# christophersanborn/Radiative3D

Hardware: AMD Instinct MI355X
Metric: phonon-histories/sec (higher is better)
Workload: dtype f64

## Files before the change

### radiative3d_amd/csrc/r3d_tables_build.h

```cpp
#ifndef R3D_TABLES_BUILD_H_
#define R3D_TABLES_BUILD_H_

#include <hip/hip_runtime.h>

#include <cstdint>

#include "r3d_tables.h"

namespace r3d {

hipError_t build_scatterer_tables(const double het[6], double psdf_numer, const double* d_toa, uint64_t n,
                                  double* d_cdf[4], double* d_spol, double totals[4], double cos_sums[4],
                                  hipStream_t stream);

hipError_t build_toa_on_device(int degree, uint64_t n, double* d_toa, hipStream_t stream);
hipError_t build_toa_xyz_on_device(const double* d_toa, uint64_t n, double min_theta, double max_theta,
                                   double* d_xyz, hipStream_t stream);
hipError_t build_source_tables(const double moment[6], const double* d_toa, uint64_t n, double* d_cdf[3],
                               double totals[3], hipStream_t stream);

hipError_t build_spol_cs_on_device(const double* d_spol, uint64_t n, double* d_cs, hipStream_t stream);

hipError_t build_guide_on_device(const double* d_cdf, uint64_t n, uint32_t bits, GuideCell* d_guide,
                                 hipStream_t stream);

}
#endif
```

### radiative3d_amd/csrc/r3d_tables_build.hip

```cpp
#include <hip/hip_runtime.h>

#include <cmath>
#include <cstdint>
#include <vector>

#include "r3d_tables_build.h"

namespace r3d {

namespace {

constexpr int kThreads = 256;
constexpr int kItems = 16;
constexpr int kScanBlock = kThreads * kItems;

struct Het {
  double nu, eps, a, kappa, el, gam0, psdf_numer;
};

__device__ __forceinline__ double psato(const Het& h, double m) {
  return h.psdf_numer / pow(1. + h.a * h.a * m * m, h.kappa + 1.5);
}

__global__ __launch_bounds__(kThreads) void gsato_kernel(Het h, const double* __restrict__ toa, uint64_t n,
                                                         double* __restrict__ w0, double* __restrict__ w1,
                                                         double* __restrict__ w2, double* __restrict__ w3,
                                                         double* __restrict__ spol,
                                                         double* __restrict__ block_cos ) {
  const uint64_t k = (uint64_t)blockIdx.x * kThreads + threadIdx.x;
  double g[4] = {0, 0, 0, 0}, cz = 0;
  if (k < n) {
    const double psi = toa[2 * k], zeta = toa[2 * k + 1];
    const double g2 = h.gam0 * h.gam0;
    const double cpsi = cos(psi), c2psi = cos(2. * psi), spsi = sin(psi);
    const double czeta = cos(zeta), szeta = sin(zeta);
    const double spsi2 = spsi * spsi;
    const double xpp = (1. / g2) * (h.nu * (-1. + cpsi + (2. / g2) * spsi2) - 2. + (4. / g2) * spsi2);
    const double xps = -spsi * (h.nu * (1. - (2. / h.gam0) * cpsi) - (4. / h.gam0) * cpsi);
    const double xsp = (1. / g2) * spsi * czeta * (h.nu * (1. - (2. / h.gam0) * cpsi) - (4. / h.gam0) * cpsi);
    const double xss_psi = czeta * (h.nu * (cpsi - c2psi) - 2. * c2psi);
    const double xss_zeta = szeta * (h.nu * (cpsi - 1.) + 2. * cpsi);
    const double pi4 = 4. * 3.14159265358979323846;
    const double el4 = (h.el * h.el) * (h.el * h.el);
    double m = (2. * h.el / h.gam0) * sin(psi / 2.);
    g[0] = (el4 / pi4) * (xpp * xpp) * psato(h, m);
    m = (h.el / h.gam0) * sqrt(1. + g2 - 2. * h.gam0 * cpsi);
    const double pm = psato(h, m);
    g[1] = (1. / h.gam0) * (el4 / pi4) * (xps * xps) * pm;
    g[2] = h.gam0 * (el4 / pi4) * (xsp * xsp) * pm;
    m = 2. * h.el * sin(psi / 2.);
    g[3] = (el4 / pi4) * (xss_psi * xss_psi + xss_zeta * xss_zeta) * psato(h, m);
#pragma unroll
    for (int c = 0; c < 4; c++)
      if (g[c] < 1.e-30) g[c] = 0.;
    w0[k] = g[0], w1[k] = g[1], w2[k] = g[2], w3[k] = g[3];
    spol[k] = atan2(xss_zeta, xss_psi);
    cz = cpsi;
  }
  __shared__ double s_part[kThreads / 64][4];
#pragma unroll
  for (int c = 0; c < 4; c++) {
    double v = cz * g[c];
#pragma unroll
    for (int off = 32; off > 0; off >>= 1) v += __shfl_xor(v, off);
    if ((threadIdx.x & 63) == 0) s_part[threadIdx.x >> 6][c] = v;
  }
  __syncthreads();
  if (threadIdx.x < 4) {
    double v = 0;
    for (int wv = 0; wv < kThreads / 64; wv++) v += s_part[wv][threadIdx.x];
    block_cos[(size_t)blockIdx.x * 4 + threadIdx.x] = v;
  }
}

__global__ __launch_bounds__(kThreads) void scan_blocks(double* const* __restrict__ arrays, uint64_t n,
                                                        double* __restrict__ block_sums, uint32_t n_blocks) {
  double* v = arrays[blockIdx.y];
  const uint64_t base = (uint64_t)blockIdx.x * kScanBlock + (uint64_t)threadIdx.x * kItems;
  double x[kItems];
  double run = 0;
#pragma unroll
  for (int i = 0; i < kItems; i++) {
    const uint64_t k = base + i;
    run += (k < n) ? v[k] : 0.0;
    x[i] = run;
  }
  __shared__ double s_run[kThreads];
  s_run[threadIdx.x] = run;
  __syncthreads();
  if (threadIdx.x == 0) {
    double acc = 0;
    for (int t = 0; t < kThreads; t++) {
      const double r = s_run[t];
      s_run[t] = acc;
      acc += r;
    }
  }
  __syncthreads();
  const double before = s_run[threadIdx.x];
#pragma unroll
  for (int i = 0; i < kItems; i++) {
    const uint64_t k = base + i;
    if (k < n) v[k] = before + x[i];
  }
  if (threadIdx.x == kThreads - 1) block_sums[(size_t)blockIdx.y * n_blocks + blockIdx.x] = before + run;
}

__global__ void scan_block_sums(double* __restrict__ block_sums, uint32_t n_blocks) {
  double* s = block_sums + (size_t)blockIdx.x * n_blocks;
  if (threadIdx.x == 0) {
    double run = 0;
    for (uint32_t b = 0; b < n_blocks; b++) {
      const double t = s[b];
      s[b] = run;
      run += t;
    }
  }
}

__global__ __launch_bounds__(kThreads) void add_offsets(double* const* __restrict__ arrays, uint64_t n,
                                                        const double* __restrict__ block_sums, uint32_t n_blocks) {
  double* v = arrays[blockIdx.y];
  const double off = block_sums[(size_t)blockIdx.y * n_blocks + blockIdx.x];
  if (blockIdx.x == 0) return;
  const uint64_t base = (uint64_t)blockIdx.x * kScanBlock;
  for (int i = threadIdx.x; i < kScanBlock; i += kThreads) {
    const uint64_t k = base + i;
    if (k < n) v[k] += off;
  }
}

__device__ uint64_t guide_bound(const double* __restrict__ cdf, uint64_t n, uint64_t j, uint64_t G) {
  const double r = cdf[n - 1] * ((double)j / (double)G);
  uint64_t lo = 0, hi = n - 1;
  while (lo < hi) {
    const uint64_t mid = (lo + hi) >> 1;
    if (r <= cdf[mid]) hi = mid;
    else lo = mid + 1;
  }
  return lo;
}
__global__ __launch_bounds__(kThreads) void guide_kernel(const double* __restrict__ cdf, uint64_t n, uint32_t bits,
                                                         GuideCell* __restrict__ guide) {
  const uint64_t G = 1ull << bits;
  const uint64_t j = (uint64_t)blockIdx.x * kThreads + threadIdx.x;
  if (j >= G) return;
  GuideCell c;
  const uint64_t k1 = guide_bound(cdf, n, j, G), k2 = guide_bound(cdf, n, j + 1, G);
  c.k1 = (uint32_t)k1, c.k2 = (uint32_t)k2;
#pragma unroll
  for (int i = 0; i < kGuideVals; i++)
    c.c[i] = (k2 - k1 <= (uint64_t)kGuideVals) ? cdf[k1 + i < k2 ? k1 + i : k2] : cdf[guide_pivot(k1, k2, i)];
  guide[j] = c;
}

struct P3 {
  double x, y, z;
};
__device__ __forceinline__ P3 unit_sum2(P3 a, P3 b) {
#pragma clang fp contract(off)
  const double sx = a.x + b.x, sy = a.y + b.y, sz = a.z + b.z;
  const double m = sqrt(sx * sx + sy * sy + sz * sz);
  return P3{sx / m, sy / m, sz / m};
}
__global__ __launch_bounds__(kThreads) void toa_kernel(int degree, uint64_t n, double* __restrict__ toa) {
#pragma clang fp contract(off)
  const uint64_t k = (uint64_t)blockIdx.x * kThreads + threadIdx.x;
  if (k >= n) return;
  const double g = (1. + sqrt(5.0)) / 2.0;
  const double m1 = sqrt(1.0 + g * g);
  const double u = 1.0 / m1, w = g / m1;
  const P3 v[12] = {{u, 0, w},  {-u, 0, w}, {u, 0, -w}, {-u, 0, -w}, {w, -u, 0}, {w, u, 0},
                    {-w, -u, 0}, {-w, u, 0}, {0, w, u},  {0, w, -u},  {0, -w, u}, {0, -w, -u}};
  const int face[20][3] = {{0, 1, 10}, {0, 1, 8},  {2, 3, 11}, {2, 3, 9},  {4, 5, 0},  {4, 5, 2},  {7, 6, 1},
                           {7, 6, 3},  {10, 11, 4}, {10, 11, 6}, {8, 9, 5},  {8, 9, 7},  {0, 10, 4}, {0, 8, 5},
                           {1, 10, 6}, {1, 8, 7},  {2, 11, 4}, {2, 9, 5},  {3, 11, 6}, {3, 9, 7}};
  const uint32_t f = (uint32_t)(k >> (2 * degree));
  P3 a = v[face[f][0]], b = v[face[f][1]], c = v[face[f][2]];
  for (int level = degree - 1; level >= 0; level--) {
    const uint32_t d = (uint32_t)(k >> (2 * level)) & 3u;
    const P3 ab = unit_sum2(a, b), bc = unit_sum2(b, c), ca = unit_sum2(c, a);
    if (d == 0) b = ab, c = ca;
    else if (d == 1) a = ab, c = bc;
    else if (d == 2) a = ca, b = bc;
    else a = bc, b = ca, c = ab;
  }
  const double sx = a.x + b.x + c.x, sy = a.y + b.y + c.y, sz = a.z + b.z + c.z;
  const double m = sqrt(sx * sx + sy * sy + sz * sz);
  toa[2 * k] = acos(sz / m);
  toa[2 * k + 1] = atan2(sy / m, sx / m);
}
__global__ __launch_bounds__(kThreads) void toa_xyz_kernel(const double* __restrict__ toa, uint64_t n, double min_theta,
                                                           double max_theta, double* __restrict__ xyz) {
#pragma clang fp contract(off)
  const uint64_t k = (uint64_t)blockIdx.x * kThreads + threadIdx.x;
  if (k >= n) return;
  double th = toa[2 * k];
  const double ph = toa[2 * k + 1];
  if (th < min_theta) th = min_theta;
  if (th > max_theta) th = max_theta;
  xyz[4 * k] = cos(th), xyz[4 * k + 1] = cos(ph), xyz[4 * k + 2] = sin(ph), xyz[4 * k + 3] = sin(th);
}
struct Moment {
  double xx, yy, zz, xy, xz, yz;
};
__global__ __launch_bounds__(kThreads) void source_kernel(Moment mt, const double* __restrict__ toa, uint64_t n,
                                                          double* __restrict__ w0, double* __restrict__ w1,
                                                          double* __restrict__ w2) {
  const uint64_t k = (uint64_t)blockIdx.x * kThreads + threadIdx.x;
  if (k >= n) return;
  const double th = toa[2 * k], az = toa[2 * k + 1];
  const double st = sin(th), ct = cos(th), sa = sin(az), ca = cos(az);
  const double horiz = mt.xx * ca * ca + mt.xy * sin(2 * az) + mt.yy * sa * sa - mt.zz;
  const double vert = mt.xz * ca + mt.yz * sa;
  const double p = st * st * horiz + 2 * st * ct * vert + mt.zz;
  const double sh = st * (0.5 * sin(2 * az) * (mt.yy - mt.xx) + cos(2 * az) * mt.xy) + ct * (ca * mt.yz - sa * mt.xz);
  const double sv = st * ct * horiz + (1.0 - 2 * st * st) * vert;
  w0[k] = p * p, w1[k] = sh * sh, w2[k] = sv * sv;
}

hipError_t scan_arrays(double* const* d_arr, int count, uint64_t n, hipStream_t stream) {
  const uint32_t s_blocks = (uint32_t)((n + kScanBlock - 1) / kScanBlock);
  double* d_sums = nullptr;
  double** d_arrays = nullptr;
  hipError_t err = hipMalloc(&d_sums, (size_t)s_blocks * count * sizeof(double));
  if (err == hipSuccess) err = hipMalloc(&d_arrays, count * sizeof(double*));
  if (err == hipSuccess) err = hipMemcpyAsync(d_arrays, d_arr, count * sizeof(double*), hipMemcpyHostToDevice, stream);
  if (err == hipSuccess) {
    scan_blocks<<<dim3(s_blocks, count), kThreads, 0, stream>>>(d_arrays, n, d_sums, s_blocks);
    scan_block_sums<<<count, 64, 0, stream>>>(d_sums, s_blocks);
    add_offsets<<<dim3(s_blocks, count), kThreads, 0, stream>>>(d_arrays, n, d_sums, s_blocks);
    err = hipGetLastError();
  }
  if (err == hipSuccess) err = hipStreamSynchronize(stream);
  (void)hipFree(d_sums), (void)hipFree(d_arrays);
  return err;
}

}

hipError_t build_toa_on_device(int degree, uint64_t n, double* d_toa, hipStream_t stream) {
  if (degree < 0 || degree > 12 || n != ((uint64_t)20 << (2 * degree))) return hipErrorInvalidValue;
  toa_kernel<<<(uint32_t)((n + kThreads - 1) / kThreads), kThreads, 0, stream>>>(degree, n, d_toa);
  return hipGetLastError();
}

hipError_t build_toa_xyz_on_device(const double* d_toa, uint64_t n, double min_theta, double max_theta,
                                   double* d_xyz, hipStream_t stream) {
  toa_xyz_kernel<<<(uint32_t)((n + kThreads - 1) / kThreads), kThreads, 0, stream>>>(d_toa, n, min_theta, max_theta, d_xyz);
  return hipGetLastError();
}

hipError_t build_source_tables(const double moment[6], const double* d_toa, uint64_t n, double* d_cdf[3],
                               double totals[3], hipStream_t stream) {
  if (n == 0) return hipErrorInvalidValue;
  const Moment mt{moment[0], moment[1], moment[2], moment[3], moment[4], moment[5]};
  source_kernel<<<(uint32_t)((n + kThreads - 1) / kThreads), kThreads, 0, stream>>>(mt, d_toa, n, d_cdf[0], d_cdf[1], d_cdf[2]);
  hipError_t err = hipGetLastError();
  if (err == hipSuccess) err = scan_arrays(d_cdf, 3, n, stream);
  for (int c = 0; c < 3 && err == hipSuccess; c++)
    err = hipMemcpy(&totals[c], d_cdf[c] + (n - 1), sizeof(double), hipMemcpyDeviceToHost);
  return err;
}

hipError_t build_scatterer_tables(const double het[6], double psdf_numer, const double* d_toa, uint64_t n,
                                  double* d_cdf[4], double* d_spol, double totals[4], double cos_sums[4],
                                  hipStream_t stream) {
  if (n == 0) return hipErrorInvalidValue;
  Het h{het[0], het[1], het[2], het[3], het[4], het[5], psdf_numer};
  const uint32_t g_blocks = (uint32_t)((n + kThreads - 1) / kThreads);
  const uint32_t s_blocks = (uint32_t)((n + kScanBlock - 1) / kScanBlock);
  double *d_cos = nullptr, *d_sums = nullptr;
  double** d_arrays = nullptr;
  hipError_t err = hipMalloc(&d_cos, (size_t)g_blocks * 4 * sizeof(double));
  if (err == hipSuccess) err = hipMalloc(&d_sums, (size_t)s_blocks * 4 * sizeof(double));
  if (err == hipSuccess) err = hipMalloc(&d_arrays, 4 * sizeof(double*));
  if (err == hipSuccess) err = hipMemcpyAsync(d_arrays, d_cdf, 4 * sizeof(double*), hipMemcpyHostToDevice, stream);
  if (err == hipSuccess) {
    gsato_kernel<<<g_blocks, kThreads, 0, stream>>>(h, d_toa, n, d_cdf[0], d_cdf[1], d_cdf[2], d_cdf[3], d_spol, d_cos);
    scan_blocks<<<dim3(s_blocks, 4), kThreads, 0, stream>>>(d_arrays, n, d_sums, s_blocks);
    scan_block_sums<<<4, 64, 0, stream>>>(d_sums, s_blocks);
    add_offsets<<<dim3(s_blocks, 4), kThreads, 0, stream>>>(d_arrays, n, d_sums, s_blocks);
    err = hipGetLastError();
  }
  std::vector<double> h_cos((size_t)g_blocks * 4);
  if (err == hipSuccess)
    err = hipMemcpyAsync(h_cos.data(), d_cos, h_cos.size() * sizeof(double), hipMemcpyDeviceToHost, stream);
  for (int c = 0; c < 4 && err == hipSuccess; c++)
    err = hipMemcpyAsync(&totals[c], d_cdf[c] + (n - 1), sizeof(double), hipMemcpyDeviceToHost, stream);
  if (err == hipSuccess) err = hipStreamSynchronize(stream);
  if (err == hipSuccess) {
    for (int c = 0; c < 4; c++) cos_sums[c] = 0;
    for (uint32_t b = 0; b < g_blocks; b++)
      for (int c = 0; c < 4; c++) cos_sums[c] += h_cos[(size_t)b * 4 + c];
  }
  (void)hipFree(d_cos), (void)hipFree(d_sums), (void)hipFree(d_arrays);
  return err;
}

__global__ __launch_bounds__(kThreads) void spol_cs_kernel(const double* __restrict__ spol, uint64_t n,
                                                           double* __restrict__ cs) {
  const uint64_t k = (uint64_t)blockIdx.x * kThreads + threadIdx.x;
  if (k >= n) return;
  double s, c;
  sincos(spol[k], &s, &c);
  cs[2 * k] = c, cs[2 * k + 1] = s;
}
hipError_t build_spol_cs_on_device(const double* d_spol, uint64_t n, double* d_cs, hipStream_t stream) {
  spol_cs_kernel<<<(uint32_t)((n + kThreads - 1) / kThreads), kThreads, 0, stream>>>(d_spol, n, d_cs);
  return hipGetLastError();
}

hipError_t build_guide_on_device(const double* d_cdf, uint64_t n, uint32_t bits, GuideCell* d_guide,
                                 hipStream_t stream) {
  const uint64_t G = 1ull << bits;
  guide_kernel<<<(uint32_t)((G + kThreads - 1) / kThreads), kThreads, 0, stream>>>(d_cdf, n, bits, d_guide);
  return hipGetLastError();
}

}
```

Measured before the change: 1.388 billion.

## Restructure table-build scan and guide construction with LDS staging and wave-parallel search

Replaces the three-kernel scan (local scan, serial block-sum scan, add offsets) with a reduce-then-scan scheme. Loads are coalesced and staged through padded LDS, block offsets come from an LDS-chunked serial chain, and array pointers travel by value instead of through a device copy. The guide builder now locates segment bounds with a 64-lane ballot search, samples the CDF segment into LDS, and writes cells with coalesced 16-byte stores. Host-side syncs and per-total memcpys are merged into one readback. This only touches table setup, so its effect on a histories/sec throughput metric depends on whether setup time is inside the timed region.

```diff
diff --git a/radiative3d_amd/csrc/r3d_tables_build.h b/radiative3d_amd/csrc/r3d_tables_build.h
--- a/radiative3d_amd/csrc/r3d_tables_build.h
+++ b/radiative3d_amd/csrc/r3d_tables_build.h
@@ -19,6 +19,8 @@
 hipError_t build_source_tables(const double moment[6], const double* d_toa, uint64_t n, double* d_cdf[3],
                                double totals[3], hipStream_t stream);
 
+hipError_t scan_arrays(double* const* d_arr, int count, uint64_t n, hipStream_t stream);
+
 hipError_t build_spol_cs_on_device(const double* d_spol, uint64_t n, double* d_cs, hipStream_t stream);
 
 hipError_t build_guide_on_device(const double* d_cdf, uint64_t n, uint32_t bits, GuideCell* d_guide,
diff --git a/radiative3d_amd/csrc/r3d_tables_build.hip b/radiative3d_amd/csrc/r3d_tables_build.hip
--- a/radiative3d_amd/csrc/r3d_tables_build.hip
+++ b/radiative3d_amd/csrc/r3d_tables_build.hip
@@ -73,85 +73,181 @@
   }
 }
 
-__global__ __launch_bounds__(kThreads) void scan_blocks(double* const* __restrict__ arrays, uint64_t n,
-                                                        double* __restrict__ block_sums, uint32_t n_blocks) {
-  double* v = arrays[blockIdx.y];
-  const uint64_t base = (uint64_t)blockIdx.x * kScanBlock + (uint64_t)threadIdx.x * kItems;
-  double x[kItems];
+struct ScanArrays {
+  double* v[4];
+};
+constexpr int kScanPad = kScanBlock + kScanBlock / kItems;
+__device__ __forceinline__ int scan_slot(int e) { return e + (e >> 4); }
+
+__device__ __forceinline__ double chain_in_lds(double* s, uint32_t m, double run) {
+  double cur[8], nxt[8];
+#pragma unroll
+  for (int i = 0; i < 8; i++) cur[i] = s[i];
+  for (uint32_t b = 0; b < m; b += 8) {
+#pragma unroll
+    for (int i = 0; i < 8; i++) nxt[i] = s[b + 8 + i];
+#pragma unroll
+    for (int i = 0; i < 8; i++) {
+      s[b + i] = run;
+      run += cur[i];
+      cur[i] = nxt[i];
+    }
+  }
+  return run;
+}
+
+__device__ __forceinline__ double scan_block_runs(const double* __restrict__ v, uint64_t n, double* s_x, double* s_run,
+                                                  double* total) {
+  const uint64_t base = (uint64_t)blockIdx.x * kScanBlock;
+#pragma unroll
+  for (int i = 0; i < kItems; i++) {
+    const int e = i * kThreads + (int)threadIdx.x;
+    const uint64_t k = base + e;
+    s_x[scan_slot(e)] = (k < n) ? v[k] : 0.0;
+  }
+  __syncthreads();
   double run = 0;
 #pragma unroll
+  for (int i = 0; i < kItems; i++) run += s_x[scan_slot((int)threadIdx.x * kItems + i)];
+  s_run[threadIdx.x] = run;
+  if (threadIdx.x < 8) s_run[kThreads + threadIdx.x] = 0;
+  __syncthreads();
+  if (threadIdx.x == 0) s_run[kThreads + 8] = chain_in_lds(s_run, kThreads, 0.0);
+  __syncthreads();
+  *total = s_run[kThreads + 8];
+  return s_run[threadIdx.x];
+}
+constexpr int kScanRun = kThreads + 8 + 1;
+
+__global__ __launch_bounds__(kThreads) void scan_block_totals(ScanArrays a, uint64_t n, double* __restrict__ block_sums,
+                                                              uint32_t n_blocks) {
+  __shared__ double s_x[kScanPad];
+  __shared__ double s_run[kScanRun];
+  double total;
+  (void)scan_block_runs(a.v[blockIdx.y], n, s_x, s_run, &total);
+  if (threadIdx.x == 0) block_sums[(size_t)blockIdx.y * n_blocks + blockIdx.x] = total;
+}
+
+__global__ __launch_bounds__(kThreads) void scan_block_offsets(double* __restrict__ block_sums, uint32_t n_blocks) {
+  __shared__ double s_t[kScanBlock + 16];
+  __shared__ double s_carry;
+  double* s = block_sums + (size_t)blockIdx.x * n_blocks;
+  if (threadIdx.x == 0) s_carry = 0;
+  for (uint32_t first = 0; first < n_blocks; first += kScanBlock) {
+    const uint32_t m = n_blocks - first < (uint32_t)kScanBlock ? n_blocks - first : (uint32_t)kScanBlock;
+    for (uint32_t i = threadIdx.x; i < m; i += kThreads) s_t[i] = s[first + i];
+    if (threadIdx.x < 16) s_t[m + threadIdx.x] = 0;
+    __syncthreads();
+    if (threadIdx.x == 0) s_carry = chain_in_lds(s_t, m, s_carry);
+    __syncthreads();
+    for (uint32_t i = threadIdx.x; i < m; i += kThreads) s[first + i] = s_t[i];
+    __syncthreads();
+  }
+}
+
+__global__ __launch_bounds__(kThreads) void scan_apply(ScanArrays a, uint64_t n, const double* __restrict__ block_offsets,
+                                                       uint32_t n_blocks, double* __restrict__ last) {
+  __shared__ double s_x[kScanPad];
+  __shared__ double s_run[kScanRun];
+  double* v = a.v[blockIdx.y];
+  double total;
+  const double before = scan_block_runs(v, n, s_x, s_run, &total);
+  const double off = block_offsets[(size_t)blockIdx.y * n_blocks + blockIdx.x];
+  double run = 0;
+#pragma unroll
   for (int i = 0; i < kItems; i++) {
-    const uint64_t k = base + i;
-    run += (k < n) ? v[k] : 0.0;
-    x[i] = run;
-  }
-  __shared__ double s_run[kThreads];
-  s_run[threadIdx.x] = run;
-  __syncthreads();
-  if (threadIdx.x == 0) {
-    double acc = 0;
-    for (int t = 0; t < kThreads; t++) {
-      const double r = s_run[t];
-      s_run[t] = acc;
-      acc += r;
+    const int slot = scan_slot((int)threadIdx.x * kItems + i);
+    run += s_x[slot];
+    double y = before + run;
+    if (blockIdx.x != 0) y += off;
+    s_x[slot] = y;
+  }
+  __syncthreads();
+  const uint64_t base = (uint64_t)blockIdx.x * kScanBlock;
+#pragma unroll
+  for (int i = 0; i < kItems; i++) {
+    const int e = i * kThreads + (int)threadIdx.x;
+    const uint64_t k = base + e;
+    if (k < n) {
+      const double y = s_x[scan_slot(e)];
+      v[k] = y;
+      if (last && k == n - 1) last[blockIdx.y] = y;
     }
   }
-  __syncthreads();
-  const double before = s_run[threadIdx.x];
-#pragma unroll
-  for (int i = 0; i < kItems; i++) {
-    const uint64_t k = base + i;
-    if (k < n) v[k] = before + x[i];
-  }
-  if (threadIdx.x == kThreads - 1) block_sums[(size_t)blockIdx.y * n_blocks + blockIdx.x] = before + run;
-}
-
-__global__ void scan_block_sums(double* __restrict__ block_sums, uint32_t n_blocks) {
-  double* s = block_sums + (size_t)blockIdx.x * n_blocks;
-  if (threadIdx.x == 0) {
-    double run = 0;
-    for (uint32_t b = 0; b < n_blocks; b++) {
-      const double t = s[b];
-      s[b] = run;
-      run += t;
-    }
-  }
-}
-
-__global__ __launch_bounds__(kThreads) void add_offsets(double* const* __restrict__ arrays, uint64_t n,
-                                                        const double* __restrict__ block_sums, uint32_t n_blocks) {
-  double* v = arrays[blockIdx.y];
-  const double off = block_sums[(size_t)blockIdx.y * n_blocks + blockIdx.x];
-  if (blockIdx.x == 0) return;
-  const uint64_t base = (uint64_t)blockIdx.x * kScanBlock;
-  for (int i = threadIdx.x; i < kScanBlock; i += kThreads) {
-    const uint64_t k = base + i;
-    if (k < n) v[k] += off;
-  }
-}
-
-__device__ uint64_t guide_bound(const double* __restrict__ cdf, uint64_t n, uint64_t j, uint64_t G) {
-  const double r = cdf[n - 1] * ((double)j / (double)G);
+}
+
+__device__ __forceinline__ double guide_level(const double* __restrict__ cdf, uint64_t n, uint64_t j, uint64_t G) {
+  return cdf[n - 1] * ((double)j / (double)G);
+}
+__device__ uint64_t guide_bound_wave(const double* __restrict__ cdf, uint64_t n, double r) {
+  const uint32_t lane = threadIdx.x & 63u;
   uint64_t lo = 0, hi = n - 1;
   while (lo < hi) {
-    const uint64_t mid = (lo + hi) >> 1;
-    if (r <= cdf[mid]) hi = mid;
-    else lo = mid + 1;
+    const uint64_t step = ((hi - lo) >> 6) + 1;
+    const uint64_t probe = lo + (uint64_t)(lane + 1) * step - 1;
+    const bool found = probe >= hi || r <= cdf[probe];
+    const uint32_t first = (uint32_t)__ffsll((unsigned long long)__ballot(found)) - 1u;
+    const uint64_t at = lo + (uint64_t)(first + 1) * step - 1;
+    if (first > 0) lo = at - step + 1;
+    hi = at < hi ? at : hi;
   }
   return lo;
 }
-__global__ __launch_bounds__(kThreads) void guide_kernel(const double* __restrict__ cdf, uint64_t n, uint32_t bits,
-                                                         GuideCell* __restrict__ guide) {
+constexpr int kGuideSeg = kThreads * (int)(sizeof(GuideCell) / sizeof(double));
+__global__ __launch_bounds__(kThreads) void guide_cells_kernel(const double* __restrict__ cdf, uint64_t n, uint32_t bits,
+                                                               GuideCell* __restrict__ guide) {
+  __shared__ uint64_t s_bound[kThreads + 1];
+  __shared__ GuideCell s_cell[kThreads];
+  double* const s_seg = reinterpret_cast<double*>(s_cell);
   const uint64_t G = 1ull << bits;
-  const uint64_t j = (uint64_t)blockIdx.x * kThreads + threadIdx.x;
-  if (j >= G) return;
+  const uint64_t j0 = (uint64_t)blockIdx.x * kThreads;
+  const uint32_t cells = G - j0 < (uint64_t)kThreads ? (uint32_t)(G - j0) : (uint32_t)kThreads;
+  const uint32_t wave = threadIdx.x >> 6;
+  if (wave < 2) {
+    const uint64_t j = wave == 0 ? j0 : j0 + cells;
+    const uint64_t k = guide_bound_wave(cdf, n, guide_level(cdf, n, j, G));
+    if ((threadIdx.x & 63u) == 0) s_bound[wave == 0 ? 0 : cells] = k;
+  }
+  __syncthreads();
+  const uint64_t first = s_bound[0], last = s_bound[cells];
+  const uint64_t len = last - first + 1;
+  const uint64_t stride = (len + kGuideSeg - 1) / kGuideSeg;
+  const uint32_t m = (uint32_t)((len + stride - 1) / stride);
+  for (uint32_t i = threadIdx.x; i < m; i += kThreads) s_seg[i] = cdf[first + i * stride];
+  __syncthreads();
+  if (threadIdx.x > 0 && threadIdx.x < cells) {
+    const double r = guide_level(cdf, n, j0 + threadIdx.x, G);
+    uint32_t a = 0, b = m;
+    while (a < b) {
+      const uint32_t mid = (a + b) >> 1;
+      if (r <= s_seg[mid]) b = mid;
+      else a = mid + 1;
+    }
+    uint64_t lo = a == 0 ? first : first + (uint64_t)(a - 1) * stride + 1;
+    uint64_t hi = a < m ? first + (uint64_t)a * stride : last;
+    while (lo < hi) {
+      const uint64_t mid = (lo + hi) >> 1;
+      if (r <= cdf[mid]) hi = mid;
+      else lo = mid + 1;
+    }
+    s_bound[threadIdx.x] = lo;
+  }
+  __syncthreads();
   GuideCell c;
-  const uint64_t k1 = guide_bound(cdf, n, j, G), k2 = guide_bound(cdf, n, j + 1, G);
-  c.k1 = (uint32_t)k1, c.k2 = (uint32_t)k2;
-#pragma unroll
-  for (int i = 0; i < kGuideVals; i++)
-    c.c[i] = (k2 - k1 <= (uint64_t)kGuideVals) ? cdf[k1 + i < k2 ? k1 + i : k2] : cdf[guide_pivot(k1, k2, i)];
-  guide[j] = c;
+  if (threadIdx.x < cells) {
+    const uint64_t k1 = s_bound[threadIdx.x], k2 = s_bound[threadIdx.x + 1];
+    auto entry = [&](uint64_t k) { return stride == 1 ? s_seg[k - first] : cdf[k]; };
+    c.k1 = (uint32_t)k1, c.k2 = (uint32_t)k2;
+#pragma unroll
+    for (int i = 0; i < kGuideVals; i++)
+      c.c[i] = (k2 - k1 <= (uint64_t)kGuideVals) ? entry(k1 + i < k2 ? k1 + i : k2) : entry(guide_pivot(k1, k2, i));
+  }
+  __syncthreads();
+  if (threadIdx.x < cells) s_cell[threadIdx.x] = c;
+  __syncthreads();
+  const uint4* src = reinterpret_cast<const uint4*>(s_cell);
+  uint4* dst = reinterpret_cast<uint4*>(guide + j0);
+  for (uint32_t i = threadIdx.x; i < cells * (uint32_t)(sizeof(GuideCell) / sizeof(uint4)); i += kThreads) dst[i] = src[i];
 }
 
 struct P3 {
@@ -219,24 +315,36 @@
   w0[k] = p * p, w1[k] = sh * sh, w2[k] = sv * sv;
 }
 
+struct Scratch {
+  void* p = nullptr;
+  ~Scratch() {
+    if (p) (void)hipFree(p);
+  }
+  hipError_t alloc(size_t doubles) { return hipMalloc(&p, doubles * sizeof(double)); }
+  double* d() const { return static_cast<double*>(p); }
+};
+
+uint32_t scan_blocks_of(uint64_t n) { return (uint32_t)((n + kScanBlock - 1) / kScanBlock); }
+
+hipError_t enqueue_scan(double* const* d_arr, int count, uint64_t n, double* d_sums, double* d_last, hipStream_t stream) {
+  ScanArrays a{};
+  for (int c = 0; c < count; c++) a.v[c] = d_arr[c];
+  const uint32_t s_blocks = scan_blocks_of(n);
+  scan_block_totals<<<dim3(s_blocks, count), kThreads, 0, stream>>>(a, n, d_sums, s_blocks);
+  scan_block_offsets<<<count, kThreads, 0, stream>>>(d_sums, s_blocks);
+  scan_apply<<<dim3(s_blocks, count), kThreads, 0, stream>>>(a, n, d_sums, s_blocks, d_last);
+  return hipGetLastError();
+}
+
+}
+
 hipError_t scan_arrays(double* const* d_arr, int count, uint64_t n, hipStream_t stream) {
-  const uint32_t s_blocks = (uint32_t)((n + kScanBlock - 1) / kScanBlock);
-  double* d_sums = nullptr;
-  double** d_arrays = nullptr;
-  hipError_t err = hipMalloc(&d_sums, (size_t)s_blocks * count * sizeof(double));
-  if (err == hipSuccess) err = hipMalloc(&d_arrays, count * sizeof(double*));
-  if (err == hipSuccess) err = hipMemcpyAsync(d_arrays, d_arr, count * sizeof(double*), hipMemcpyHostToDevice, stream);
-  if (err == hipSuccess) {
-    scan_blocks<<<dim3(s_blocks, count), kThreads, 0, stream>>>(d_arrays, n, d_sums, s_blocks);
-    scan_block_sums<<<count, 64, 0, stream>>>(d_sums, s_blocks);
-    add_offsets<<<dim3(s_blocks, count), kThreads, 0, stream>>>(d_arrays, n, d_sums, s_blocks);
-    err = hipGetLastError();
-  }
-  if (err == hipSuccess) err = hipStreamSynchronize(stream);
-  (void)hipFree(d_sums), (void)hipFree(d_arrays);
+  if (n == 0 || count < 1 || count > 4 || !d_arr) return hipErrorInvalidValue;
+  Scratch scratch;
+  hipError_t err = scratch.alloc((size_t)scan_blocks_of(n) * count);
+  if (err == hipSuccess) err = enqueue_scan(d_arr, count, n, scratch.d(), nullptr, stream);
+  if (hipError_t f = hipStreamSynchronize(stream); err == hipSuccess) err = f;
   return err;
-}
-
 }
 
 hipError_t build_toa_on_device(int degree, uint64_t n, double* d_toa, hipStream_t stream) {
@@ -255,11 +363,16 @@
                                double totals[3], hipStream_t stream) {
   if (n == 0) return hipErrorInvalidValue;
   const Moment mt{moment[0], moment[1], moment[2], moment[3], moment[4], moment[5]};
-  source_kernel<<<(uint32_t)((n + kThreads - 1) / kThreads), kThreads, 0, stream>>>(mt, d_toa, n, d_cdf[0], d_cdf[1], d_cdf[2]);
-  hipError_t err = hipGetLastError();
-  if (err == hipSuccess) err = scan_arrays(d_cdf, 3, n, stream);
-  for (int c = 0; c < 3 && err == hipSuccess; c++)
-    err = hipMemcpy(&totals[c], d_cdf[c] + (n - 1), sizeof(double), hipMemcpyDeviceToHost);
+  const size_t n_sums = (size_t)scan_blocks_of(n) * 3;
+  Scratch scratch;
+  hipError_t err = scratch.alloc(n_sums + 3);
+  if (err == hipSuccess) {
+    source_kernel<<<(uint32_t)((n + kThreads - 1) / kThreads), kThreads, 0, stream>>>(mt, d_toa, n, d_cdf[0], d_cdf[1], d_cdf[2]);
+    err = enqueue_scan(d_cdf, 3, n, scratch.d(), scratch.d() + n_sums, stream);
+  }
+  if (err == hipSuccess)
+    err = hipMemcpyAsync(totals, scratch.d() + n_sums, 3 * sizeof(double), hipMemcpyDeviceToHost, stream);
+  if (hipError_t f = hipStreamSynchronize(stream); err == hipSuccess) err = f;
   return err;
 }
 
@@ -269,32 +382,23 @@
   if (n == 0) return hipErrorInvalidValue;
   Het h{het[0], het[1], het[2], het[3], het[4], het[5], psdf_numer};
   const uint32_t g_blocks = (uint32_t)((n + kThreads - 1) / kThreads);
-  const uint32_t s_blocks = (uint32_t)((n + kScanBlock - 1) / kScanBlock);
-  double *d_cos = nullptr, *d_sums = nullptr;
-  double** d_arrays = nullptr;
-  hipError_t err = hipMalloc(&d_cos, (size_t)g_blocks * 4 * sizeof(double));
-  if (err == hipSuccess) err = hipMalloc(&d_sums, (size_t)s_blocks * 4 * sizeof(double));
-  if (err == hipSuccess) err = hipMalloc(&d_arrays, 4 * sizeof(double*));
-  if (err == hipSuccess) err = hipMemcpyAsync(d_arrays, d_cdf, 4 * sizeof(double*), hipMemcpyHostToDevice, stream);
+  const size_t n_cos = (size_t)g_blocks * 4, n_sums = (size_t)scan_blocks_of(n) * 4;
+  Scratch scratch;
+  hipError_t err = scratch.alloc(n_cos + 4 + n_sums);
+  double* const d_cos = scratch.d();
   if (err == hipSuccess) {
     gsato_kernel<<<g_blocks, kThreads, 0, stream>>>(h, d_toa, n, d_cdf[0], d_cdf[1], d_cdf[2], d_cdf[3], d_spol, d_cos);
-    scan_blocks<<<dim3(s_blocks, 4), kThreads, 0, stream>>>(d_arrays, n, d_sums, s_blocks);
-    scan_block_sums<<<4, 64, 0, stream>>>(d_sums, s_blocks);
-    add_offsets<<<dim3(s_blocks, 4), kThreads, 0, stream>>>(d_arrays, n, d_sums, s_blocks);
-    err = hipGetLastError();
-  }
-  std::vector<double> h_cos((size_t)g_blocks * 4);
+    err = enqueue_scan(d_cdf, 4, n, d_cos + n_cos + 4, d_cos + n_cos, stream);
+  }
+  std::vector<double> h_back(n_cos + 4);
   if (err == hipSuccess)
-    err = hipMemcpyAsync(h_cos.data(), d_cos, h_cos.size() * sizeof(double), hipMemcpyDeviceToHost, stream);
-  for (int c = 0; c < 4 && err == hipSuccess; c++)
-    err = hipMemcpyAsync(&totals[c], d_cdf[c] + (n - 1), sizeof(double), hipMemcpyDeviceToHost, stream);
-  if (err == hipSuccess) err = hipStreamSynchronize(stream);
+    err = hipMemcpyAsync(h_back.data(), d_cos, h_back.size() * sizeof(double), hipMemcpyDeviceToHost, stream);
+  if (hipError_t f = hipStreamSynchronize(stream); err == hipSuccess) err = f;
   if (err == hipSuccess) {
-    for (int c = 0; c < 4; c++) cos_sums[c] = 0;
+    for (int c = 0; c < 4; c++) cos_sums[c] = 0, totals[c] = h_back[n_cos + c];
     for (uint32_t b = 0; b < g_blocks; b++)
-      for (int c = 0; c < 4; c++) cos_sums[c] += h_cos[(size_t)b * 4 + c];
-  }
-  (void)hipFree(d_cos), (void)hipFree(d_sums), (void)hipFree(d_arrays);
+      for (int c = 0; c < 4; c++) cos_sums[c] += h_back[(size_t)b * 4 + c];
+  }
   return err;
 }
 
@@ -314,7 +418,7 @@
 hipError_t build_guide_on_device(const double* d_cdf, uint64_t n, uint32_t bits, GuideCell* d_guide,
                                  hipStream_t stream) {
   const uint64_t G = 1ull << bits;
-  guide_kernel<<<(uint32_t)((G + kThreads - 1) / kThreads), kThreads, 0, stream>>>(d_cdf, n, bits, d_guide);
+  guide_cells_kernel<<<(uint32_t)((G + kThreads - 1) / kThreads), kThreads, 0, stream>>>(d_cdf, n, bits, d_guide);
   return hipGetLastError();
 }
 
```

Result: no change. 1.390 billion (median of 3 runs) (+0.1%).
